# FutureSDR/FutureSDR

Hardware: NVIDIA H100
Metric: Msamples/s (higher is better)
Workload: dtype f32

## Files before the change

### futuresdr_b200/_lib.py

```python
from __future__ import annotations

import ctypes as C
import os

_HERE = os.path.dirname(os.path.abspath(__file__))
SO_PATH = os.environ.get("B2S_LIB") or os.path.join(_HERE, "libb200sdr.so")

OK, EINVAL, ECUDA, ENOMEM, EAGAIN, EUNSUPPORTED, ESTATE, ETIMEOUT = 0, -1, -2, -3, -4, -5, -6, -7
INSUFFICIENT_INPUT, INSUFFICIENT_OUTPUT, BOTH_SUFFICIENT = 0, 1, 2
F32_F32, C32_F32, C32_C32, F64_F64 = 0, 1, 2, 3
ALGO_AUTO, ALGO_DIRECT, ALGO_TENSOR, ALGO_FFT, ALGO_SCAN = 0, 1, 2, 3, 4
(OP_SCALE_F32, OP_SCALE_C32, OP_QUAD_DEMOD, OP_NORM_SQR, OP_QUAD_DEMOD_C32, OP_EXP_F32,
 OP_MAG_C32, OP_LOG10_F32, OP_DC_BLOCK_F32, OP_SLICE_F32_U8) = range(10)
KEYFOB_NONE, KEYFOB_CLOSE, KEYFOB_OPEN, KEYFOB_TRUNK = 0, 1, 2, 3
WAVE_COS, WAVE_SIN, WAVE_SQUARE = 0, 1, 2
(COMBINE_ADD_F32, COMBINE_SUB_F32, COMBINE_MUL_F32, COMBINE_CONJ_MUL_C32, COMBINE_MAG_DIV_C32_F32, COMBINE_TO_C32,
 COMBINE_TO_C32_NEG_Q) = range(7)
SPLIT_RE_IM, SPLIT_DUP_F32 = 0, 1
FANOUT_MAX_OUTPUTS = 256

_vp, _sz, _i32, _f32 = C.c_void_p, C.c_size_t, C.c_int32, C.c_float
_szp, _i32p, _vpp, _f32p = C.POINTER(C.c_size_t), C.POINTER(C.c_int32), C.POINTER(C.c_void_p), C.POINTER(C.c_float)

SIGNATURES = {
    "b2s_version": (_i32, []),
    "b2s_ctx_create": (_i32, [C.c_int, _vpp]),
    "b2s_ctx_create_on_stream": (_i32, [C.c_int, _vp, _vpp]),
    "b2s_ctx_destroy": (None, [_vp]),
    "b2s_last_error": (C.c_char_p, [_vp]),
    "b2s_ctx_sync": (_i32, [_vp]),
    "b2s_ctx_stream": (_vp, [_vp]),
    "b2s_ctx_sm_count": (_i32, [_vp]),
    "b2s_ctx_launch_count": (C.c_uint64, [_vp]),
    "b2s_ctx_bytes_held": (C.c_uint64, [_vp]),
    "b2s_malloc": (_i32, [_vp, _sz, _vpp]),
    "b2s_free": (_i32, [_vp, _vp]),
    "b2s_host_alloc": (_i32, [_vp, _sz, _vpp]),
    "b2s_host_free": (_i32, [_vp, _vp]),
    "b2s_memcpy_h2d": (_i32, [_vp, _vp, _vp, _sz]),
    "b2s_memcpy_d2h": (_i32, [_vp, _vp, _vp, _sz]),
    "b2s_fir_plan": (_i32, [_vp, C.c_int, _f32p, _sz, _sz, _vpp]),
    "b2s_fir_plan_f32_f32": (_i32, [_vp, _f32p, _sz, _sz, _vpp]),
    "b2s_fir_plan_c32_f32": (_i32, [_vp, _f32p, _sz, _sz, _vpp]),
    "b2s_fir_plan_c32_c32": (_i32, [_vp, _f32p, _sz, _sz, _vpp]),
    "b2s_fir_plan_f64_f64": (_i32, [_vp, C.POINTER(C.c_double), _sz, _sz, _vpp]),
    "b2s_fir_destroy": (None, [_vp]),
    "b2s_fir_length": (_sz, [_vp]),
    "b2s_fir_set_algo": (_i32, [_vp, C.c_int]),
    "b2s_fir_get_algo": (_i32, [_vp]),
    "b2s_fir_exec": (_i32, [_vp, _vp, _sz, _vp, _sz, _szp, _szp, _i32p]),
    "b2s_fir_filter_host": (_i32, [_vp, _vp, _sz, _vp, _sz, _szp, _szp, _i32p]),
    "b2s_fir_exec_hist": (_i32, [_vp, _vp, _sz, _vp, _sz, _vp, _sz, _vp, _szp, _szp, _i32p]),
    "b2s_resamp_plan": (_i32, [_vp, C.c_int, _f32p, _sz, _sz, _sz, _vpp]),
    "b2s_resamp_destroy": (None, [_vp]),
    "b2s_resamp_length": (_sz, [_vp]),
    "b2s_resamp_exec": (_i32, [_vp, _vp, _sz, _vp, _sz, _szp, _szp, _i32p]),
    "b2s_pfbarb_plan_c32": (_i32, [_vp, _f32p, _sz, _sz, _f32, _vpp]),
    "b2s_pfbarb_destroy": (None, [_vp]),
    "b2s_pfbarb_reset": (_i32, [_vp]),
    "b2s_pfbarb_period": (_i32, [_f32, _sz, C.POINTER(C.c_uint64), C.POINTER(C.c_uint64)]),
    "b2s_pfbarb_exec": (_i32, [_vp, _vp, _sz, _vp, _sz, _szp, _szp, _i32p]),
    "b2s_fft_plan_c32": (_i32, [_vp, _sz, _i32, _i32, _i32, _f32, _vpp]),
    "b2s_fft_destroy": (None, [_vp]),
    "b2s_fft_length": (_sz, [_vp]),
    "b2s_fft_exec": (_i32, [_vp, _vp, _sz, _vp, _sz, _szp, _szp]),
    "b2s_apply_create": (_i32, [_vp, C.c_int, _f32, _vpp]),
    "b2s_apply_destroy": (None, [_vp]),
    "b2s_apply_reset": (_i32, [_vp]),
    "b2s_apply_exec": (_i32, [_vp, _vp, _sz, _vp, _sz, _szp, _szp]),
    "b2s_rotator_create": (_i32, [_vp, _f32, _vpp]),
    "b2s_rotator_destroy": (None, [_vp]),
    "b2s_rotator_reset": (_i32, [_vp]),
    "b2s_rotator_exec": (_i32, [_vp, _vp, _sz, _vp, _sz, _szp, _i32p]),
    "b2s_xlating_taps": (_i32, [_f32p, _sz, _f32, _f32, _sz, _f32p, _f32p]),
    "b2s_chan_plan_c32": (_i32, [_vp, _sz, _f32p, _sz, _f32, _vpp]),
    "b2s_chan_destroy": (None, [_vp]),
    "b2s_chan_decimation": (_sz, [_vp]),
    "b2s_chan_exec": (_i32, [_vp, _vp, _sz, _vp, _sz, _sz, _szp, _szp, _i32p]),
    "b2s_synth_plan_c32": (_i32, [_vp, _sz, _f32p, _sz, _vpp]),
    "b2s_synth_destroy": (None, [_vp]),
    "b2s_synth_exec": (_i32, [_vp, _vp, _sz, _sz, _vp, _sz, _szp, _szp]),
    "b2s_mavg_create": (_i32, [_vp, _sz, _f32, _sz, _vpp]),
# ... 137 lines not shown
```

### futuresdr_b200/csrc/abi.cu

```cuda
#include <cmath>
#include <cstdlib>
#include <memory>

#include "fir.cuh"

thread_local std::string g_b2s_last_error;

int32_t b2s_fail(b2s_ctx *ctx, int32_t code, const char *fmt, ...) {
    char buf[512];
    va_list ap;
    va_start(ap, fmt);
    vsnprintf(buf, sizeof(buf), fmt, ap);
    va_end(ap);
    g_b2s_last_error = buf;
    if (ctx) ctx->err = buf;
    return code;
}

extern "C" {

int32_t b2s_version(void) { return B2S_VERSION; }

static int32_t ctx_create(int device, void *stream, bool own, b2s_ctx **out) {
    if (!out) return b2s_fail(nullptr, B2S_EINVAL, "b2s_ctx_create: out is NULL");
// ... 181 lines not shown
}
int32_t b2s_fir_plan_c32_f32(b2s_ctx *c, const float *t, size_t n, size_t d, b2s_fir **o) {
    return b2s_fir_plan(c, B2S_C32_F32, t, n, d, o);
}
int32_t b2s_fir_plan_c32_c32(b2s_ctx *c, const float *t, size_t n, size_t d, b2s_fir **o) {
    return b2s_fir_plan(c, B2S_C32_C32, t, n, d, o);
}

void b2s_fir_destroy(b2s_fir *f) { PlanDeleter<b2s_fir>()(f); }

size_t b2s_fir_length(const b2s_fir *f) { return f ? f->ntaps : 0; }

int32_t b2s_fir_set_algo(b2s_fir *f, b2s_algo algo) {
    if (!f) return b2s_fail(nullptr, B2S_EINVAL, "fir is NULL");
    if (algo < B2S_ALGO_AUTO || algo > B2S_ALGO_FFT)
        return b2s_fail(f->ctx, B2S_EUNSUPPORTED, "FIR filters have the AUTO, DIRECT, TENSOR and FFT algorithms (got %d)", (int)algo);
    if (f->kind == B2S_F64_F64)
        return algo == B2S_ALGO_AUTO || algo == B2S_ALGO_DIRECT ? B2S_OK
               : b2s_fail(f->ctx, B2S_EUNSUPPORTED, "f64 filters only have the CUDA-core form");
    if (algo == B2S_ALGO_TENSOR && !fir_tc_supported(f))
        return b2s_fail(f->ctx, B2S_EUNSUPPORTED,
                        "tensor algorithm needs real taps, 16..257 of them, and a decimation that divides 128 (kind %d, ntaps %zu, decim %zu)",
                        (int)f->kind, f->ntaps, f->decim);
    if (algo == B2S_ALGO_FFT && !fir_fft_supported(f))
        return b2s_fail(f->ctx, B2S_EUNSUPPORTED,
                        "FFT algorithm needs Complex<f32> samples, 64..2049 taps and decim == 1 (kind %d, ntaps %zu, decim %zu)",
                        (int)f->kind, f->ntaps, f->decim);
    f->algo_req = algo;
    resolve_algo(f);
    DeviceGuard g(f->ctx->device);
    return prepare_algo(f);
}
int32_t b2s_fir_get_algo(const b2s_fir *f) { return f ? (int32_t)f->algo : B2S_EINVAL; }

static void fir_counts(const b2s_fir *f, size_t n_in, size_t n_out_cap, size_t *consumed,
                       size_t *produced, int32_t *status) {
    const size_t filterable = sat_sub(n_in + 1, f->ntaps);
    const size_t consumable = filterable / f->decim;
    size_t n;
    int32_t st;
    if (consumable > n_out_cap) { n = n_out_cap; st = B2S_INSUFFICIENT_OUTPUT; }
    else if (consumable == n_out_cap) { n = n_out_cap; st = B2S_BOTH_SUFFICIENT; }
    else { n = consumable; st = B2S_INSUFFICIENT_INPUT; }
    *consumed = n * f->decim; *produced = n; *status = st;
}

static int32_t fir_launch(b2s_fir *f, const void *d_in, size_t n_in, void *d_out, size_t n_out,
                          cudaStream_t stream) {
    if (f->kind == B2S_F64_F64) return fir_f64_launch(f, d_in, n_in, d_out, n_out, stream);
    if (f->algo == B2S_ALGO_TENSOR && f->algo_req == B2S_ALGO_AUTO) {
        const double per_tap = f->kind == B2S_F32_F32 ? 6.9e-14 : 1.15e-13;
        if ((double)n_out * (double)f->ntaps * per_tap < 10e-6) return fir_direct_launch(f, d_in, n_in, d_out, n_out, stream);
    }
    if (f->algo == B2S_ALGO_TENSOR) return fir_tc_launch(f, d_in, n_in, d_out, n_out, stream);
    if (f->algo == B2S_ALGO_FFT) return fir_fft_launch(f, d_in, n_in, d_out, n_out, stream);
    return fir_direct_launch(f, d_in, n_in, d_out, n_out, stream);
}

int32_t b2s_fir_exec(b2s_fir *f, const void *d_in, size_t n_in, void *d_out, size_t n_out_cap,
                     size_t *consumed, size_t *produced, int32_t *status) {
    if (!f || !consumed || !produced || !status)
        return b2s_fail(f ? f->ctx : nullptr, B2S_EINVAL, "b2s_fir_exec: NULL argument");
    fir_counts(f, n_in, n_out_cap, consumed, produced, status);
    if (*produced == 0) return B2S_OK;
    if (!d_in || !d_out) return b2s_fail(f->ctx, B2S_EINVAL, "b2s_fir_exec: NULL buffer");
    DeviceGuard g(f->ctx->device);
// ... 118 lines not shown
```

### futuresdr_b200/csrc/fir.cuh

```cuda
#pragma once
#include "common.cuh"

struct b2s_fir {
    b2s_ctx *ctx = nullptr;
    b2s_kind kind = B2S_C32_F32;
    size_t ntaps = 0, decim = 1;
    std::vector<float> taps_host;
    b2s_algo algo_req = B2S_ALGO_AUTO, algo = B2S_ALGO_DIRECT;

    Buf<float> d_ptaps;
    int Upad = 0;

    int tc_kblocks = 0;
    bool tc_ready = false;
    int tc_flags = 0;

    Buf<float2> d_fftH;

    Buf<double> d_taps64;
};

int32_t fir_direct_prepare(b2s_fir *f);
int32_t fir_direct_launch(b2s_fir *f, const void *d_in, size_t n_in, void *d_out, size_t n_out,
                          cudaStream_t stream);
std::vector<float> slide_table(const float *taps, size_t tf, size_t L, size_t M, size_t T, size_t lead);
bool    resamp_slide_supported(size_t L, size_t M, size_t T, size_t item_bytes);
int32_t resamp_slide_launch(b2s_ctx *ctx, b2s_kind kind, const float *d_gtab, size_t L, size_t M, size_t T,
                            const void *d_in, size_t n_in, void *d_out, size_t n_out, cudaStream_t stream);
struct FirHist {
    const void *d_hist = nullptr;
    size_t n_hist = 0;
    unsigned *publish_flag = nullptr;
    unsigned publish_value = 0;
    const unsigned *wait_flag = nullptr;
    unsigned wait_value = 0;
    unsigned *done_flag = nullptr;
    unsigned done_value = 0;
};
bool    fir_tc_supported(const b2s_fir *f);
int32_t fir_tc_launch_hist(b2s_fir *f, const FirHist *h, const void *d_in, size_t n_in, void *d_out, size_t n_out,
                           cudaStream_t stream);
int32_t fir_tc_prepare(b2s_fir *f);
int32_t fir_tc_launch(b2s_fir *f, const void *d_in, size_t n_in, void *d_out, size_t n_out,
                      cudaStream_t stream);
int32_t fir_f64_prepare(b2s_fir *f, const double *taps);
int32_t fir_f64_launch(b2s_fir *f, const void *d_in, size_t n_in, void *d_out, size_t n_out, cudaStream_t stream);
bool    fir_fft_supported(const b2s_fir *f);
int32_t fir_fft_prepare(b2s_fir *f);
int32_t fir_fft_launch(b2s_fir *f, const void *d_in, size_t n_in, void *d_out, size_t n_out,
                       cudaStream_t stream);
```

### futuresdr_b200/csrc/fir_tc.cu

```cuda
#include <cuda_bf16.h>

#include <algorithm>
#include <climits>
#include <cstdlib>
#include <type_traits>

#include "fir.cuh"

namespace {

constexpr int kStages = 2;
#ifndef B2S_RAW_SLOTS
#define B2S_RAW_SLOTS 6
#endif
constexpr int kRawSlots = B2S_RAW_SLOTS;
constexpr int kRawSlotBytes = 8192;
constexpr int kNumProducerThreads = 256;
constexpr int kNumMathThreads = 256;
constexpr int kNumLoaderThreads = 128;
constexpr int kThreadsTC = kNumMathThreads + kNumProducerThreads + kNumLoaderThreads;
constexpr int kProdWarps = kNumProducerThreads / 32;
constexpr int kMathWarps = kNumMathThreads / 32;
constexpr int kProdWarp0 = kMathWarps;
constexpr int kTmaWarp = kProdWarp0 + kProdWarps;
constexpr int kRegsAtLaunch = 65536 / kThreadsTC / 8 * 8;
constexpr int kMathRegs = 176, kProdRegs = 48, kLoaderRegs = 24;
static_assert(kNumMathThreads * kMathRegs + kNumProducerThreads * kProdRegs + kNumLoaderThreads * kLoaderRegs <=
              kThreadsTC * kRegsAtLaunch, "setmaxnreg budget exceeds the CTA's register allocation");
constexpr int kAtomsOut = 16;
constexpr int kMaxDK = 3;
constexpr int kMaxKSteps = (63 + 128 * kMaxDK - 128) / 16 + 1;
constexpr int kSplitBytesMax = (kAtomsOut + kMaxDK - 1) * 1024 * 2;
constexpr int kStageBytes = 2 * kSplitBytesMax;
constexpr int kACores = kMaxDK * 16 + 15;
constexpr int kABytes = kACores * 128;
constexpr int kSmemTC = kStages * kStageBytes + kRawSlots * kRawSlotBytes + 2 * kABytes + 1024  + 256 ;
static_assert(kSmemTC <= 227 * 1024, "tensor FIR shared memory exceeds the 227 KiB per-CTA limit");

__device__ __forceinline__ uint32_t smem_u32(const void *p) { return (uint32_t)__cvta_generic_to_shared(p); }

__device__ __forceinline__ void mbar_init(uint32_t bar, uint32_t count) {
    asm volatile("mbarrier.init.shared::cta.b64 [%0], %1;" ::"r"(bar), "r"(count));
}
__device__ __forceinline__ void mbar_arrive(uint32_t bar) {
    asm volatile("mbarrier.arrive.shared::cta.b64 _, [%0];" ::"r"(bar) : "memory");
}
__device__ __forceinline__ bool mbar_try_wait(uint32_t bar, uint32_t parity) {
    uint32_t ok;
    asm volatile(
        "{\n\t.reg .pred p;\n\t"
        "mbarrier.try_wait.parity.shared::cta.b64 p, [%1], %2;\n\t"
        "selp.b32 %0, 1, 0, p;\n\t}"
        : "=r"(ok) : "r"(bar), "r"(parity) : "memory");
    return ok != 0;
}
__device__ __forceinline__ void mbar_wait(uint32_t bar, uint32_t parity) {
    while (!mbar_try_wait(bar, parity)) {}
}
__device__ __forceinline__ bool elect_one() {
    uint32_t pred;
    asm volatile("{\n\t.reg .pred p;\n\telect.sync _|p, 0xffffffff;\n\tselp.b32 %0, 1, 0, p;\n\t}" : "=r"(pred));
    return pred != 0;
}
__device__ __forceinline__ void fence_barrier_init() { asm volatile("fence.mbarrier_init.release.cluster;" ::: "memory"); }
__device__ __forceinline__ void fence_proxy_async() { asm volatile("fence.proxy.async.shared::cta;" ::: "memory"); }

__device__ __forceinline__ void wgmma_fence() { asm volatile("wgmma.fence.sync.aligned;" ::: "memory"); }
__device__ __forceinline__ void wgmma_commit() { asm volatile("wgmma.commit_group.sync.aligned;" ::: "memory"); }
__device__ __forceinline__ void wgmma_wait_all() { asm volatile("wgmma.wait_group.sync.aligned 0;" ::: "memory"); }
// ... 42 lines not shown
          "+f"(d[16]), "+f"(d[17]), "+f"(d[18]), "+f"(d[19]), "+f"(d[20]), "+f"(d[21]), "+f"(d[22]), "+f"(d[23]),
          "+f"(d[24]), "+f"(d[25]), "+f"(d[26]), "+f"(d[27]), "+f"(d[28]), "+f"(d[29]), "+f"(d[30]), "+f"(d[31]),
          "+f"(d[32]), "+f"(d[33]), "+f"(d[34]), "+f"(d[35]), "+f"(d[36]), "+f"(d[37]), "+f"(d[38]), "+f"(d[39]),
          "+f"(d[40]), "+f"(d[41]), "+f"(d[42]), "+f"(d[43]), "+f"(d[44]), "+f"(d[45]), "+f"(d[46]), "+f"(d[47]),
          "+f"(d[48]), "+f"(d[49]), "+f"(d[50]), "+f"(d[51]), "+f"(d[52]), "+f"(d[53]), "+f"(d[54]), "+f"(d[55]),
          "+f"(d[56]), "+f"(d[57]), "+f"(d[58]), "+f"(d[59]), "+f"(d[60]), "+f"(d[61]), "+f"(d[62]), "+f"(d[63])
        : "r"(a[0]), "r"(a[1]), "r"(a[2]), "r"(a[3]), "l"(b_desc), "r"(accumulate)
        : "memory");
}
__device__ __forceinline__ uint32_t ld_shared_b32(uint32_t addr) {
    uint32_t v;
    asm volatile("ld.shared.b32 %0, [%1];" : "=r"(v) : "r"(addr));
    return v;
}

__device__ __forceinline__ uint32_t cvt_bf16x2(float a, float b) {
    uint32_t r;
    asm("cvt.rn.bf16x2.f32 %0, %1, %2;" : "=r"(r) : "f"(b), "f"(a));
    return r;
}
__device__ __forceinline__ void split2(float a, float b, uint32_t &hi, uint32_t &lo) {
    hi = cvt_bf16x2(a, b);
    const float ah = __uint_as_float(hi << 16), bh = __uint_as_float(hi & 0xffff0000u);
    lo = cvt_bf16x2(a - ah, b - bh);
}

__device__ __forceinline__ uint64_t make_desc(uint32_t smem_addr, uint32_t lbo, uint32_t sbo, uint32_t layout) {
    return (uint64_t)((smem_addr & 0x3FFFF) >> 4) | ((uint64_t)(lbo >> 4) << 16) | ((uint64_t)(sbo >> 4) << 32) |
           ((uint64_t)layout << 62);
}
__device__ __forceinline__ uint64_t make_b_desc(uint32_t smem_addr) { return make_desc(smem_addr, 16, 1024, 1); }
__device__ __forceinline__ uint64_t make_a_desc(uint32_t smem_addr) { return make_desc(smem_addr, 128, 128, 0); }

struct TcParams {
    const float *in;
    float *out;
    const float *g;
    long long n_in;
    long long n_out;
    int ntaps;
    int DK;
    int num_tiles;
    int flags;
    int decim;
    const float *hist;
    int hist_items;
    int lead;
    const unsigned *wait_flag;
    unsigned wait_value;
    unsigned *done_flag;
    unsigned done_value;
    unsigned *pub_flag;
    unsigned pub_value;
    unsigned *status;
};

template <bool COMPLEX>
__global__ void __launch_bounds__(kThreadsTC, 1) fir_tc_kernel(const TcParams prm) {
    extern __shared__ unsigned char smem_raw[];
    const uint32_t raw = smem_u32(smem_raw);
    const uint32_t base = (raw + 1023u) & ~1023u;
    unsigned char *gen_base = smem_raw + (base - raw);
    const uint32_t raw_base = base + kStages * kStageBytes;
    unsigned char *raw_gen = gen_base + kStages * kStageBytes;
    const uint32_t a_base = raw_base + kRawSlots * kRawSlotBytes;
    __nv_bfloat16 *a_gen = reinterpret_cast<__nv_bfloat16 *>(raw_gen + kRawSlots * kRawSlotBytes);
    const uint32_t bar_base = a_base + 2 * kABytes;
    auto full_bar = [&](int s) { return bar_base + 8u * s; };
    auto empty_bar = [&](int s) { return bar_base + 8u * (kStages + s); };
    auto rfull_bar = [&](int r) { return bar_base + 8u * (2 * kStages + r); };
    auto rempty_bar = [&](int r) { return bar_base + 8u * (2 * kStages + kRawSlots + r); };

    const int warp = threadIdx.x >> 5, lane = threadIdx.x & 31;
    if (prm.pub_flag && blockIdx.x == 0 && threadIdx.x == 0) {
        __threadfence_system();
        asm volatile("st.release.sys.global.u32 [%0], %1;" ::"l"(prm.pub_flag), "r"(prm.pub_value) : "memory");
    }
    const int DK = prm.DK, K = 128 * DK;
    const int atoms = kAtomsOut + DK - 1;
    const int chunk_bytes = atoms * 1024;
    const int split_bytes = 2 * chunk_bytes;
    constexpr int NSEQ = COMPLEX ? 4 : 8;
    constexpr int TILE_BLOCKS = kAtomsOut * NSEQ;
    constexpr long long TILE_ITEMS = (long long)TILE_BLOCKS * 128;

    if (warp == kTmaWarp && lane == 0) {
        for (int s = 0; s < kStages; s++) { mbar_init(full_bar(s), kProdWarps); mbar_init(empty_bar(s), kMathWarps); }
        for (int r = 0; r < kRawSlots; r++) { mbar_init(rfull_bar(r), 1); mbar_init(rempty_bar(r), kProdWarps); }
        fence_barrier_init();
    }
    const int a_elems = (K / 8 + 15) * 64;
    for (int i = threadIdx.x; i < a_elems; i += kThreadsTC) {
        const int s = i >> 6, r = (i >> 3) & 7, e = i & 7;
        const int t = 8 * s + r + e - 127 - prm.lead;
        const float gv = (t >= 0 && t < prm.ntaps) ? __ldg(prm.g + t) : 0.0f;
        const __nv_bfloat16 hi = __float2bfloat16_rn(gv);
        a_gen[i] = hi;
        a_gen[kABytes / 2 + i] = __float2bfloat16_rn(gv - __bfloat162float(hi));
    }
    fence_proxy_async();
    __syncthreads();

    constexpr int F4_PER_BLOCK = COMPLEX ? 64 : 32;
    constexpr int BLOCKS_PER_SLOT = 512 / F4_PER_BLOCK;
    constexpr int SLOTS_PER_TILE = (TILE_BLOCKS + kMaxDK - 1 + BLOCKS_PER_SLOT - 1) / BLOCKS_PER_SLOT;
    constexpr int ITEM_BYTES = COMPLEX ? 8 : 4;
    const int in_blocks = TILE_BLOCKS + DK - 1;

    if (warp >= kTmaWarp) {
        setmaxnreg_dec<kLoaderRegs>();
        if (warp != kTmaWarp) return;
        if (elect_one()) {
            int rs = 0;
            uint32_t rphase = 0;
            for (int tile = blockIdx.x; tile < prm.num_tiles; tile += gridDim.x) {
                const long long item0 = (long long)tile * TILE_ITEMS;
#pragma unroll 1
                for (int s = 0; s < SLOTS_PER_TILE; s++) {
                    const int blk_first = s * BLOCKS_PER_SLOT;
                    if (blk_first >= in_blocks) break;
                    const int nblk = min(BLOCKS_PER_SLOT, in_blocks - blk_first);
                    const long long it0 = item0 + (long long)blk_first * 128;
                    long long items = (long long)nblk * 128;
                    if (it0 + items > prm.n_in) items = prm.n_in - it0;
                    long long bytes = items > 0 ? ((items * ITEM_BYTES) & ~15ll) : 0;
                    mbar_wait(rempty_bar(rs), rphase ^ 1);
                    if (tile == 0 && s == 0 && prm.hist_items > 0) {
                        if (prm.wait_flag) {
                            unsigned long long t0, t1;
                            asm volatile("mov.u64 %0, %%globaltimer;" : "=l"(t0));
                            for (;;) {
                                unsigned v;
                                asm volatile("ld.acquire.sys.global.u32 %0, [%1];" : "=r"(v) : "l"(prm.wait_flag) : "memory");
                                if ((int)(v - prm.wait_value) >= 0) break;
                                asm volatile("mov.u64 %0, %%globaltimer;" : "=l"(t1));
                                if (t1 - t0 > 4000000000ull) { atomicOr(prm.status, 1u); break; }
                                __nanosleep(64);
                            }
                            asm volatile("fence.proxy.async;" ::: "memory");
                        }
                        const uint32_t hb = (uint32_t)prm.hist_items * ITEM_BYTES;
                        const uint32_t rest = bytes > (long long)hb ? (uint32_t)bytes - hb : 0u;
                        asm volatile("mbarrier.arrive.expect_tx.shared::cta.b64 _, [%0], %1;" ::"r"(rfull_bar(rs)), "r"(hb + rest) : "memory");
                        asm volatile("cp.async.bulk.shared::cluster.global.mbarrier::complete_tx::bytes [%0], [%1], %2, [%3];"
                                     ::"r"(raw_base + rs * kRawSlotBytes), "l"(prm.hist), "r"(hb), "r"(rfull_bar(rs)) : "memory");
                        if (rest)
                            asm volatile("cp.async.bulk.shared::cluster.global.mbarrier::complete_tx::bytes [%0], [%1], %2, [%3];"
                                         ::"r"(raw_base + rs * kRawSlotBytes + hb), "l"(prm.in + (COMPLEX ? 2 : 1) * (long long)prm.hist_items),
                                           "r"(rest), "r"(rfull_bar(rs)) : "memory");
                    } else if (bytes > 0) {
                        asm volatile("mbarrier.arrive.expect_tx.shared::cta.b64 _, [%0], %1;" ::"r"(rfull_bar(rs)), "r"((uint32_t)bytes) : "memory");
                        asm volatile("cp.async.bulk.shared::cluster.global.mbarrier::complete_tx::bytes [%0], [%1], %2, [%3];"
                                     ::"r"(raw_base + rs * kRawSlotBytes), "l"(prm.in + (COMPLEX ? 2 : 1) * it0),
                                       "r"((uint32_t)bytes), "r"(rfull_bar(rs)) : "memory");
                    } else {
                        mbar_arrive(rfull_bar(rs));
                    }
                    if (++rs == kRawSlots) { rs = 0; rphase ^= 1; }
                }
            }
        }
        __syncwarp();
    } else if (warp >= kProdWarp0) {
        setmaxnreg_dec<kProdRegs>();
        const int tid = threadIdx.x - 32 * kProdWarp0;
        const int fo = tid % F4_PER_BLOCK, rowsel = tid / F4_PER_BLOCK;
        const int kc = COMPLEX ? (fo >> 5) : (fo >> 4);
        const int c16 = COMPLEX ? ((fo & 31) >> 2) : ((fo & 15) >> 1);
        const int wofs = COMPLEX ? (fo & 3) * 4 : (fo & 1) * 8;
        const uint32_t t_off = (uint32_t)(kc * chunk_bytes + wofs + rowsel * 1024);
        uint32_t xj[8];
#pragma unroll
        for (int j = 0; j < 8; j++) xj[j] = (uint32_t)(j * 128 + ((c16 ^ j) << 4));
        const bool alias_thread = rowsel < DK - 1;
        const uint32_t sb = (uint32_t)split_bytes;

        auto convert_tile = [&](auto interior_c, unsigned char *stage_ptr, long long item0, int &rs, uint32_t &rphase) {
            constexpr bool INTERIOR = decltype(interior_c)::value;
            unsigned char *tp = stage_ptr + t_off;
#pragma unroll
            for (int s = 0; s < SLOTS_PER_TILE; s++) {
                if (s * BLOCKS_PER_SLOT >= in_blocks) break;
                mbar_wait(rfull_bar(rs), rphase);
                const float4 *raw = reinterpret_cast<const float4 *>(raw_gen + rs * kRawSlotBytes);
                float4 v[2];
                v[0] = raw[tid];
                v[1] = raw[tid + 256];
                const int rs_cur = rs;
                if (++rs == kRawSlots) { rs = 0; rphase ^= 1; }
                if constexpr (!INTERIOR) {
                    if (s == 0 && item0 == 0 && tid == 0 && prm.done_flag)
// ... 33 lines not shown
                            *reinterpret_cast<uint32_t *>(q + xj[2 * (seq & 3) + 1]) = ih;
                            *reinterpret_cast<uint32_t *>(q + xj[2 * (seq & 3) + 1] + sb) = il;
                        }
                        if (alias_ct && alias_thread) {
                            unsigned char *q = tp + (g_ct + kAtomsOut) * 1024;
                            *reinterpret_cast<uint32_t *>(q + xj[2 * ((seq - 1) & 3)]) = rh;
                            *reinterpret_cast<uint32_t *>(q + xj[2 * ((seq - 1) & 3)] + sb) = rl;
                            *reinterpret_cast<uint32_t *>(q + xj[2 * ((seq - 1) & 3) + 1]) = ih;
                            *reinterpret_cast<uint32_t *>(q + xj[2 * ((seq - 1) & 3) + 1] + sb) = il;
                        }
                    } else {
                        uint32_t h0, l0, h1, l1;
                        split2(v[i].x, v[i].y, h0, l0);
                        split2(v[i].z, v[i].w, h1, l1);
                        if (seq < NSEQ) {
                            unsigned char *q = tp + g_ct * 1024 + xj[seq & 7];
                            *reinterpret_cast<uint2 *>(q) = make_uint2(h0, h1);
                            *reinterpret_cast<uint2 *>(q + sb) = make_uint2(l0, l1);
                        }
                        if (alias_ct && alias_thread) {
                            unsigned char *q = tp + (g_ct + kAtomsOut) * 1024 + xj[(seq - 1) & 7];
                            *reinterpret_cast<uint2 *>(q) = make_uint2(h0, h1);
                            *reinterpret_cast<uint2 *>(q + sb) = make_uint2(l0, l1);
                        }
                    }
                }
                __syncwarp();
                if (lane == 0) mbar_arrive(rempty_bar(rs_cur));
            }
        };

        int stage = 0, rs = 0;
        uint32_t phase = 0, rphase = 0;
        for (int tile = blockIdx.x; tile < prm.num_tiles; tile += gridDim.x) {
            const long long item0 = (long long)tile * TILE_ITEMS;
            const bool interior = item0 + (long long)in_blocks * 128 <= prm.n_in &&
                                  !(tile == 0 && (prm.lead | prm.hist_items) != 0);
            mbar_wait(empty_bar(stage), phase ^ 1);
            unsigned char *stage_ptr = gen_base + stage * kStageBytes;
            if (interior) convert_tile(std::true_type{}, stage_ptr, item0, rs, rphase);
            else convert_tile(std::false_type{}, stage_ptr, item0, rs, rphase);
            fence_proxy_async();
            __syncwarp();
            if (lane == 0) mbar_arrive(full_bar(stage));
            if (++stage == kStages) { stage = 0; phase ^= 1; }
        }
    } else {
        setmaxnreg_inc<kMathRegs>();
        const int wg = __shfl_sync(0xffffffffu, warp >> 2, 0);
        const int wl = warp & 3, q4 = lane & 3;
        const int D = prm.decim, per_blk = 128 / D;
        const uint32_t a_hi = a_base + 1024u * wg, a_lo = a_hi + kABytes;
        const int p0 = 64 * (1 - wg);
        const int j0 = p0 / 16;
        const int nsteps = (prm.flags & 4) ? 0 : min((p0 + 63 + prm.lead + prm.ntaps - 1) / 16, 8 * DK - 1) - j0 + 1;

        uint32_t ghi[kMaxKSteps][4];
        {
            const uint32_t f0 = a_hi + 256u * (uint32_t)(wl + j0) + 16u * (uint32_t)(lane >> 2) + 4u * (uint32_t)q4;
#pragma unroll
            for (int i = 0; i < kMaxKSteps; i++) {
                const uint32_t f = f0 + 256u * i;
                const bool used = i < nsteps;
                ghi[i][0] = used ? ld_shared_b32(f) : 0u;
                ghi[i][1] = used ? ld_shared_b32(f + 128u) : 0u;
                ghi[i][2] = used ? ld_shared_b32(f + 128u) : 0u;
                ghi[i][3] = used ? ld_shared_b32(f + 256u) : 0u;
            }
        }

        const uint64_t a_lo_desc = make_a_desc(a_lo + 256u * j0);

        int stage = 0;
        uint32_t phase = 0;
        auto mma_tile = [&](float (&acc)[64]) {
            mbar_wait(full_bar(stage), phase);
            wgmma_fence();
            const uint64_t b_desc = make_b_desc(base + stage * kStageBytes);
#pragma unroll
            for (int i = 0; i < kMaxKSteps; i++) {
                if (i >= nsteps) break;
                const int m = (j0 >> 2) + (i >> 2);
                const uint64_t bh = b_desc + (uint32_t)(((m & 1) * chunk_bytes + (m >> 1) * 1024 + (i & 3) * 32) >> 4);
                wgmma_m64n128_rs(acc, ghi[i], bh, i != 0);
                wgmma_m64n128_rs(acc, ghi[i], bh + (uint32_t)(split_bytes >> 4), 1u);
                wgmma_m64n128(acc, a_lo_desc + 16u * i, bh, 1u);
            }
            wgmma_commit();
        };
        auto release_stage = [&]() {
            wgmma_wait_all();
            __syncwarp();
            if (lane == 0) mbar_arrive(empty_bar(stage));
            if (++stage == kStages) { stage = 0; phase ^= 1; }
        };
        const int log2D = __ffs(D) - 1;
        auto store_tile = [&](const float (&acc)[64], int tile) {
            if (prm.flags & 2) return;
#pragma unroll
            for (int h = 0; h < 2; h++) {
                const int p = 127 - (64 * wg + 16 * wl + (lane >> 2) + 8 * h);
                const int keep = (p & (D - 1)) == D - 1;
                const long long kb = ((long long)tile * TILE_BLOCKS + kAtomsOut * q4 * (COMPLEX ? 1 : 2)) * per_blk +
                                     (p >> log2D);
                const int room = (int)max(min(prm.n_out - kb, (long long)INT_MAX), 0ll) & -keep;
                const int ncols = (int)(((unsigned)room + (unsigned)per_blk - 1u) >> (7 - log2D));
                if constexpr (COMPLEX) {
#pragma unroll
                    for (int gam = 0; gam < 16; gam++)
                        st_global_if(reinterpret_cast<float2 *>(prm.out) + kb + gam * per_blk, acc[4 * gam + 2 * h],
                                     acc[4 * gam + 2 * h + 1], gam < ncols);
                } else {
#pragma unroll
                    for (int n = 0; n < 2 * kAtomsOut; n++)
                        st_global_if(prm.out + (kb + n * per_blk), acc[4 * (n % kAtomsOut) + 2 * h + n / kAtomsOut],
                                     n < ncols);
                }
            }
        };

        float acc[64];
#pragma unroll
        for (int i = 0; i < 64; i++) acc[i] = 0.0f;
        for (int tile = blockIdx.x; tile < prm.num_tiles; tile += gridDim.x) {
            mma_tile(acc);
            release_stage();
            store_tile(acc, tile);
        }
    }
}

}

bool fir_tc_supported(const b2s_fir *f) {
    if (f->decim == 0 || f->decim > 128 || 128 % f->decim != 0) return false;
    if (f->kind != B2S_C32_F32 && f->kind != B2S_F32_F32) return false;
    return f->ntaps >= 16 && f->ntaps <= 128 * kMaxDK - 127;
}

int32_t fir_tc_prepare(b2s_fir *f) {
    b2s_ctx *ctx = f->ctx;
    if (f->tc_ready) return B2S_OK;
    if (!fir_tc_supported(f)) return b2s_fail(ctx, B2S_EUNSUPPORTED, "tensor FIR: unsupported plan");
    f->tc_kblocks = (int)ceil_div(f->ntaps + 127, 128);
    B2S_CUDA(ctx, cudaFuncSetAttribute(fir_tc_kernel<true>, cudaFuncAttributeMaxDynamicSharedMemorySize, kSmemTC));
    B2S_CUDA(ctx, cudaFuncSetAttribute(fir_tc_kernel<false>, cudaFuncAttributeMaxDynamicSharedMemorySize, kSmemTC));
    for (const void *k : {(const void *)fir_tc_kernel<true>, (const void *)fir_tc_kernel<false>}) {
        cudaFuncAttributes attr;
        B2S_CUDA(ctx, cudaFuncGetAttributes(&attr, k));
        if (attr.numRegs != kRegsAtLaunch)
            return b2s_fail(ctx, B2S_EUNSUPPORTED, "tensor FIR: kernel built with %d registers per thread, its setmaxnreg "
                            "budget assumes %d", attr.numRegs, kRegsAtLaunch);
    }
    if (const char *e = getenv("B2S_TC_FLAGS")) f->tc_flags = atoi(e);
    f->tc_ready = true;
    return B2S_OK;
}

int32_t fir_tc_launch_hist(b2s_fir *f, const FirHist *h, const void *d_in, size_t n_in, void *d_out, size_t n_out,
                           cudaStream_t stream) {
    b2s_ctx *ctx = f->ctx;
    if (n_out == 0) return B2S_OK;
    if (!f->tc_ready) return b2s_fail(ctx, B2S_ESTATE, "tensor FIR not prepared");
    const bool cplx = f->kind == B2S_C32_F32;
    const size_t item = cplx ? 8 : 4, q = 16 / item;
    const uintptr_t a_in = reinterpret_cast<uintptr_t>(d_in), a_out = reinterpret_cast<uintptr_t>(d_out);
    if ((a_in % item) || (a_out % item)) return B2S_EAGAIN;
    const size_t n_hist = h ? h->n_hist : 0;
    size_t lead;
    if (n_hist) {
        const uintptr_t a_h = reinterpret_cast<uintptr_t>(h->d_hist);
        if ((a_h % item) || (a_in & 15)) return B2S_EAGAIN;
        lead = (a_h / item) % q;
        if ((lead + n_hist) % q) return B2S_EAGAIN;
        if (lead + n_hist > 1024 || n_in * item < 16) return B2S_EAGAIN;
    } else {
        lead = (a_in / item) % q;
    }
    const int DK = (int)ceil_div(f->ntaps + lead + 127, 128);
    if (DK > kMaxDK) return B2S_EAGAIN;
    TcParams prm;
    prm.lead = (int)lead;
    prm.hist_items = n_hist ? (int)(lead + n_hist) : 0;
    prm.hist = n_hist ? (const float *)h->d_hist - lead * (item / 4) : nullptr;
    prm.in = (const float *)d_in - (lead + n_hist) * (item / 4);
    prm.wait_flag = (h && n_hist) ? h->wait_flag : nullptr;
    prm.wait_value = h ? h->wait_value : 0;
    prm.done_flag = (h && n_hist) ? h->done_flag : nullptr;
    prm.done_value = h ? h->done_value : 0;
    prm.pub_flag = h ? h->publish_flag : nullptr;
    prm.pub_value = h ? h->publish_value : 0;
    prm.status = ctx->d_status;
    prm.out = (float *)d_out;
    prm.g = f->d_ptaps.get() + (size_t)f->decim * f->Upad;
    prm.n_in = (long long)(lead + n_hist + n_in);
    prm.n_out = (long long)n_out;
    prm.decim = (int)f->decim;
    prm.ntaps = (int)f->ntaps;
    prm.DK = DK;
    const long long tile_items = cplx ? 64 * 128 : 128 * 128;
    prm.num_tiles = (int)ceil_div(n_out * f->decim, (size_t)tile_items);
    prm.flags = f->tc_flags;
    const int grid = std::min(prm.num_tiles, ctx->sm_count);
    if (prm.wait_flag) ctx->flag_ops++;
    if (cplx) fir_tc_kernel<true><<<grid, kThreadsTC, kSmemTC, stream>>>(prm);
    else fir_tc_kernel<false><<<grid, kThreadsTC, kSmemTC, stream>>>(prm);
    B2S_CHECK_LAUNCH(ctx);
    return B2S_OK;
}

int32_t fir_tc_launch(b2s_fir *f, const void *d_in, size_t n_in, void *d_out, size_t n_out,
                      cudaStream_t stream) {
    const int32_t rc = fir_tc_launch_hist(f, nullptr, d_in, n_in, d_out, n_out, stream);
    if (rc == B2S_EAGAIN) return fir_direct_launch(f, d_in, n_in, d_out, n_out, stream);
    return rc;
}
```

### include/b200sdr.h

```cpp
#ifndef B200SDR_H
#define B200SDR_H

#include <stddef.h>
#include <stdint.h>

#ifdef __cplusplus
extern "C" {
#endif

#define B2S_VERSION 100

#define B2S_OK            0
#define B2S_EINVAL       (-1)
#define B2S_ECUDA        (-2)
#define B2S_ENOMEM       (-3)
#define B2S_EAGAIN       (-4)
#define B2S_EUNSUPPORTED (-5)
#define B2S_ESTATE       (-6)
#define B2S_ETIMEOUT     (-7)

#define B2S_INSUFFICIENT_INPUT  0
#define B2S_INSUFFICIENT_OUTPUT 1
#define B2S_BOTH_SUFFICIENT     2

// ... 19 lines not shown
typedef struct b2s_fft    b2s_fft;
typedef struct b2s_apply  b2s_apply;
typedef struct b2s_ring   b2s_ring;
typedef struct b2s_slot   b2s_slot;

int32_t     b2s_version(void);
int32_t     b2s_ctx_create(int device, b2s_ctx **out);
int32_t     b2s_ctx_create_on_stream(int device, void *stream, b2s_ctx **out);
void        b2s_ctx_destroy(b2s_ctx *ctx);
const char *b2s_last_error(const b2s_ctx *ctx);
int32_t     b2s_ctx_sync(b2s_ctx *ctx);
void       *b2s_ctx_stream(b2s_ctx *ctx);
int32_t     b2s_ctx_sm_count(b2s_ctx *ctx);
uint64_t    b2s_ctx_launch_count(const b2s_ctx *ctx);
uint64_t    b2s_ctx_bytes_held(const b2s_ctx *ctx);

int32_t b2s_malloc(b2s_ctx *ctx, size_t bytes, void **dptr);
int32_t b2s_free(b2s_ctx *ctx, void *dptr);
int32_t b2s_host_alloc(b2s_ctx *ctx, size_t bytes, void **hptr);
int32_t b2s_host_free(b2s_ctx *ctx, void *hptr);
int32_t b2s_memcpy_h2d(b2s_ctx *ctx, void *dptr, const void *hptr, size_t bytes);
int32_t b2s_memcpy_d2h(b2s_ctx *ctx, void *hptr, const void *dptr, size_t bytes);

int32_t b2s_fir_plan(b2s_ctx *ctx, b2s_kind kind, const float *taps, size_t ntaps, size_t decim,
                     b2s_fir **out);
int32_t b2s_fir_plan_f32_f32(b2s_ctx *ctx, const float *taps, size_t ntaps, size_t decim, b2s_fir **out);
int32_t b2s_fir_plan_c32_f32(b2s_ctx *ctx, const float *taps, size_t ntaps, size_t decim, b2s_fir **out);
int32_t b2s_fir_plan_c32_c32(b2s_ctx *ctx, const float *taps, size_t ntaps, size_t decim, b2s_fir **out);
int32_t b2s_fir_plan_f64_f64(b2s_ctx *ctx, const double *taps, size_t ntaps, size_t decim, b2s_fir **out);
void    b2s_fir_destroy(b2s_fir *f);
size_t  b2s_fir_length(const b2s_fir *f);
int32_t b2s_fir_set_algo(b2s_fir *f, b2s_algo algo);
int32_t b2s_fir_get_algo(const b2s_fir *f);

int32_t b2s_fir_exec(b2s_fir *f, const void *d_in, size_t n_in, void *d_out, size_t n_out_cap,
                     size_t *consumed, size_t *produced, int32_t *status);
typedef struct b2s_handshake {
    uint32_t       *publish_flag; uint32_t publish_value;
    const uint32_t *wait_flag;    uint32_t wait_value;
    uint32_t       *done_flag;    uint32_t done_value;
} b2s_handshake;
int32_t b2s_fir_exec_hist(b2s_fir *f, const void *d_hist, size_t n_hist, const void *d_in, size_t n_in,
                          void *d_out, size_t n_out_cap, const b2s_handshake *hs, size_t *consumed, size_t *produced,
                          int32_t *status);
int32_t b2s_fir_filter_host(b2s_fir *f, const void *h_in, size_t n_in, void *h_out, size_t n_out_cap,
                            size_t *consumed, size_t *produced, int32_t *status);

int32_t b2s_resamp_plan(b2s_ctx *ctx, b2s_kind kind, const float *taps, size_t ntaps, size_t interp,
                        size_t decim, b2s_resamp **out);
void    b2s_resamp_destroy(b2s_resamp *r);
size_t  b2s_resamp_length(const b2s_resamp *r);
int32_t b2s_resamp_exec(b2s_resamp *r, const void *d_in, size_t n_in, void *d_out, size_t n_out_cap,
                        size_t *consumed, size_t *produced, int32_t *status);

int32_t b2s_pfbarb_plan_c32(b2s_ctx *ctx, const float *taps, size_t ntaps, size_t num_filters,
                            float rate, b2s_pfbarb **out);
void    b2s_pfbarb_destroy(b2s_pfbarb *p);
int32_t b2s_pfbarb_reset(b2s_pfbarb *p);
int32_t b2s_pfbarb_period(float rate, size_t num_filters, uint64_t *period_items, uint64_t *outputs_per_period);
int32_t b2s_pfbarb_exec(b2s_pfbarb *p, const void *d_in, size_t n_in, void *d_out, size_t n_out_cap,
                        size_t *consumed, size_t *produced, int32_t *call_again);

int32_t b2s_fft_plan_c32(b2s_ctx *ctx, size_t n, int32_t inverse, int32_t fft_shift,
                         int32_t has_normalize, float normalize, b2s_fft **out);
void    b2s_fft_destroy(b2s_fft *f);
size_t  b2s_fft_length(const b2s_fft *f);
// ... 213 lines not shown
```

Before: 169,700.

## Schedule tensor FIR tiles dynamically via global atomic counter and prefetch first slots

```diff
diff --git a/futuresdr_b200/_lib.py b/futuresdr_b200/_lib.py
--- a/futuresdr_b200/_lib.py
+++ b/futuresdr_b200/_lib.py
@@ -48,6 +48,7 @@
     "b2s_fir_length": (_sz, [_vp]),
     "b2s_fir_set_algo": (_i32, [_vp, C.c_int]),
     "b2s_fir_get_algo": (_i32, [_vp]),
+    "b2s_fir_tc_timeline": (_i32, [_vp, C.POINTER(C.c_uint64), _sz, _szp]),
     "b2s_fir_exec": (_i32, [_vp, _vp, _sz, _vp, _sz, _szp, _szp, _i32p]),
     "b2s_fir_filter_host": (_i32, [_vp, _vp, _sz, _vp, _sz, _szp, _szp, _i32p]),
     "b2s_fir_exec_hist": (_i32, [_vp, _vp, _sz, _vp, _sz, _vp, _sz, _vp, _szp, _szp, _i32p]),
diff --git a/futuresdr_b200/csrc/abi.cu b/futuresdr_b200/csrc/abi.cu
--- a/futuresdr_b200/csrc/abi.cu
+++ b/futuresdr_b200/csrc/abi.cu
@@ -237,6 +237,11 @@
     return prepare_algo(f);
 }
 int32_t b2s_fir_get_algo(const b2s_fir *f) { return f ? (int32_t)f->algo : B2S_EINVAL; }
+
+int32_t b2s_fir_tc_timeline(b2s_fir *f, uint64_t *stamps, size_t cap, size_t *n_ctas) {
+    if (!f || !stamps || !n_ctas) return b2s_fail(f ? f->ctx : nullptr, B2S_EINVAL, "b2s_fir_tc_timeline: NULL argument");
+    return fir_tc_timeline(f, stamps, cap, n_ctas);
+}
 
 static void fir_counts(const b2s_fir *f, size_t n_in, size_t n_out_cap, size_t *consumed,
                        size_t *produced, int32_t *status) {
diff --git a/futuresdr_b200/csrc/fir.cuh b/futuresdr_b200/csrc/fir.cuh
--- a/futuresdr_b200/csrc/fir.cuh
+++ b/futuresdr_b200/csrc/fir.cuh
@@ -14,6 +14,9 @@
     int tc_kblocks = 0;
     bool tc_ready = false;
     int tc_flags = 0;
+    Buf<unsigned> d_tc_sched;
+    Buf<unsigned long long> d_tc_timeline;
+    int tc_timeline_ctas = 0;
 
     Buf<float2> d_fftH;
 
@@ -37,10 +40,12 @@
     unsigned *done_flag = nullptr;
     unsigned done_value = 0;
 };
+enum TcStamp { kTcEntry, kTcFirstCopy, kTcFirstFull, kTcLastTile, kTcExit, kTcTiles, kTcStampWords };
 bool    fir_tc_supported(const b2s_fir *f);
 int32_t fir_tc_launch_hist(b2s_fir *f, const FirHist *h, const void *d_in, size_t n_in, void *d_out, size_t n_out,
                            cudaStream_t stream);
 int32_t fir_tc_prepare(b2s_fir *f);
+int32_t fir_tc_timeline(b2s_fir *f, uint64_t *stamps, size_t cap, size_t *n_ctas);
 int32_t fir_tc_launch(b2s_fir *f, const void *d_in, size_t n_in, void *d_out, size_t n_out,
                       cudaStream_t stream);
 int32_t fir_f64_prepare(b2s_fir *f, const double *taps);
diff --git a/futuresdr_b200/csrc/fir_tc.cu b/futuresdr_b200/csrc/fir_tc.cu
--- a/futuresdr_b200/csrc/fir_tc.cu
+++ b/futuresdr_b200/csrc/fir_tc.cu
@@ -34,7 +34,9 @@
 constexpr int kStageBytes = 2 * kSplitBytesMax;
 constexpr int kACores = kMaxDK * 16 + 15;
 constexpr int kABytes = kACores * 128;
+constexpr int kTileRing = 8;
 constexpr int kSmemTC = kStages * kStageBytes + kRawSlots * kRawSlotBytes + 2 * kABytes + 1024  + 256 ;
+static_assert(8 * (2 * kStages + 2 * kRawSlots) + 4 * kTileRing <= 256, "barriers and tile ring exceed their 256 bytes");
 static_assert(kSmemTC <= 227 * 1024, "tensor FIR shared memory exceeds the 227 KiB per-CTA limit");
 
 __device__ __forceinline__ uint32_t smem_u32(const void *p) { return (uint32_t)__cvta_generic_to_shared(p); }
@@ -143,6 +145,12 @@
 __device__ __forceinline__ uint64_t make_b_desc(uint32_t smem_addr) { return make_desc(smem_addr, 16, 1024, 1); }
 __device__ __forceinline__ uint64_t make_a_desc(uint32_t smem_addr) { return make_desc(smem_addr, 128, 128, 0); }
 
+__device__ __forceinline__ unsigned long long globaltimer() {
+    unsigned long long t;
+    asm volatile("mov.u64 %0, %%globaltimer;" : "=l"(t));
+    return t;
+}
+
 struct TcParams {
     const float *in;
     float *out;
@@ -153,6 +161,8 @@
     int DK;
     int num_tiles;
     int flags;
+    unsigned long long *timeline;
+    unsigned *sched;
     int decim;
     const float *hist;
     int hist_items;
@@ -181,8 +191,12 @@
     auto empty_bar = [&](int s) { return bar_base + 8u * (kStages + s); };
     auto rfull_bar = [&](int r) { return bar_base + 8u * (2 * kStages + r); };
     auto rempty_bar = [&](int r) { return bar_base + 8u * (2 * kStages + kRawSlots + r); };
+    const uint32_t tile_ring = bar_base + 8u * (2 * kStages + 2 * kRawSlots);
+    auto tile_at = [&](int j) { return (int)ld_shared_b32(tile_ring + 4u * (uint32_t)(j & (kTileRing - 1))); };
 
     const int warp = threadIdx.x >> 5, lane = threadIdx.x & 31;
+    unsigned long long *const stamps = prm.timeline ? prm.timeline + (size_t)blockIdx.x * kTcStampWords : nullptr;
+    if (stamps && threadIdx.x == 0) stamps[kTcEntry] = globaltimer();
     if (prm.pub_flag && blockIdx.x == 0 && threadIdx.x == 0) {
         __threadfence_system();
         asm volatile("st.release.sys.global.u32 [%0], %1;" ::"l"(prm.pub_flag), "r"(prm.pub_value) : "memory");
@@ -195,10 +209,66 @@
     constexpr int TILE_BLOCKS = kAtomsOut * NSEQ;
     constexpr long long TILE_ITEMS = (long long)TILE_BLOCKS * 128;
 
-    if (warp == kTmaWarp && lane == 0) {
-        for (int s = 0; s < kStages; s++) { mbar_init(full_bar(s), kProdWarps); mbar_init(empty_bar(s), kMathWarps); }
-        for (int r = 0; r < kRawSlots; r++) { mbar_init(rfull_bar(r), 1); mbar_init(rempty_bar(r), kProdWarps); }
-        fence_barrier_init();
+    constexpr int F4_PER_BLOCK = COMPLEX ? 64 : 32;
+    constexpr int BLOCKS_PER_SLOT = 512 / F4_PER_BLOCK;
+    constexpr int SLOTS_PER_TILE = (TILE_BLOCKS + kMaxDK - 1 + BLOCKS_PER_SLOT - 1) / BLOCKS_PER_SLOT;
+    constexpr int ITEM_BYTES = COMPLEX ? 8 : 4;
+    const int in_blocks = TILE_BLOCKS + DK - 1;
+    const int tile_slots = (in_blocks + BLOCKS_PER_SLOT - 1) / BLOCKS_PER_SLOT;
+    const int pre_slots = min(kRawSlots, tile_slots);
+
+    auto load_slot = [&](int tile, int s, int rs, uint32_t rphase) {
+        const long long item0 = (long long)tile * TILE_ITEMS;
+        const int blk_first = s * BLOCKS_PER_SLOT;
+        const int nblk = min(BLOCKS_PER_SLOT, in_blocks - blk_first);
+        const long long it0 = item0 + (long long)blk_first * 128;
+        long long items = (long long)nblk * 128;
+        if (it0 + items > prm.n_in) items = prm.n_in - it0;
+        long long bytes = items > 0 ? ((items * ITEM_BYTES) & ~15ll) : 0;
+        mbar_wait(rempty_bar(rs), rphase ^ 1);
+        if (tile == 0 && s == 0 && prm.hist_items > 0) {
+            if (prm.wait_flag) {
+                unsigned long long t0, t1;
+                asm volatile("mov.u64 %0, %%globaltimer;" : "=l"(t0));
+                for (;;) {
+                    unsigned v;
+                    asm volatile("ld.acquire.sys.global.u32 %0, [%1];" : "=r"(v) : "l"(prm.wait_flag) : "memory");
+                    if ((int)(v - prm.wait_value) >= 0) break;
+                    asm volatile("mov.u64 %0, %%globaltimer;" : "=l"(t1));
+                    if (t1 - t0 > 4000000000ull) { atomicOr(prm.status, 1u); break; }
+                    __nanosleep(64);
+                }
+                asm volatile("fence.proxy.async;" ::: "memory");
+            }
+            const uint32_t hb = (uint32_t)prm.hist_items * ITEM_BYTES;
+            const uint32_t rest = bytes > (long long)hb ? (uint32_t)bytes - hb : 0u;
+            asm volatile("mbarrier.arrive.expect_tx.shared::cta.b64 _, [%0], %1;" ::"r"(rfull_bar(rs)), "r"(hb + rest) : "memory");
+            asm volatile("cp.async.bulk.shared::cluster.global.mbarrier::complete_tx::bytes [%0], [%1], %2, [%3];"
+                         ::"r"(raw_base + rs * kRawSlotBytes), "l"(prm.hist), "r"(hb), "r"(rfull_bar(rs)) : "memory");
+            if (rest)
+                asm volatile("cp.async.bulk.shared::cluster.global.mbarrier::complete_tx::bytes [%0], [%1], %2, [%3];"
+                             ::"r"(raw_base + rs * kRawSlotBytes + hb), "l"(prm.in + (COMPLEX ? 2 : 1) * (long long)prm.hist_items),
+                               "r"(rest), "r"(rfull_bar(rs)) : "memory");
+        } else if (bytes > 0) {
+            asm volatile("mbarrier.arrive.expect_tx.shared::cta.b64 _, [%0], %1;" ::"r"(rfull_bar(rs)), "r"((uint32_t)bytes) : "memory");
+            asm volatile("cp.async.bulk.shared::cluster.global.mbarrier::complete_tx::bytes [%0], [%1], %2, [%3];"
+                         ::"r"(raw_base + rs * kRawSlotBytes), "l"(prm.in + (COMPLEX ? 2 : 1) * it0),
+                           "r"((uint32_t)bytes), "r"(rfull_bar(rs)) : "memory");
+        } else {
+            mbar_arrive(rfull_bar(rs));
+        }
+        if (stamps && tile == blockIdx.x && s == 0) stamps[kTcFirstCopy] = globaltimer();
+    };
+
+    if (warp == kTmaWarp) {
+        if (elect_one()) {
+            for (int s = 0; s < kStages; s++) { mbar_init(full_bar(s), kProdWarps); mbar_init(empty_bar(s), kMathWarps); }
+            for (int r = 0; r < kRawSlots; r++) { mbar_init(rfull_bar(r), 1); mbar_init(rempty_bar(r), kProdWarps); }
+            fence_barrier_init();
+            asm volatile("st.shared.b32 [%0], %1;" ::"r"(tile_ring), "r"((int)blockIdx.x) : "memory");
+            for (int s = 0; s < pre_slots; s++) load_slot(blockIdx.x, s, s, 0u);
+        }
+        __syncwarp();
     }
     const int a_elems = (K / 8 + 15) * 64;
     for (int i = threadIdx.x; i < a_elems; i += kThreadsTC) {
@@ -212,62 +282,32 @@
     fence_proxy_async();
     __syncthreads();
 
-    constexpr int F4_PER_BLOCK = COMPLEX ? 64 : 32;
-    constexpr int BLOCKS_PER_SLOT = 512 / F4_PER_BLOCK;
-    constexpr int SLOTS_PER_TILE = (TILE_BLOCKS + kMaxDK - 1 + BLOCKS_PER_SLOT - 1) / BLOCKS_PER_SLOT;
-    constexpr int ITEM_BYTES = COMPLEX ? 8 : 4;
-    const int in_blocks = TILE_BLOCKS + DK - 1;
-
     if (warp >= kTmaWarp) {
         setmaxnreg_dec<kLoaderRegs>();
         if (warp != kTmaWarp) return;
         if (elect_one()) {
-            int rs = 0;
-            uint32_t rphase = 0;
-            for (int tile = blockIdx.x; tile < prm.num_tiles; tile += gridDim.x) {
-                const long long item0 = (long long)tile * TILE_ITEMS;
+            int rs = pre_slots % kRawSlots;
+            uint32_t rphase = pre_slots / kRawSlots;
+            for (int j = 0, tile = blockIdx.x, s0 = pre_slots;; s0 = 0) {
+                const int next = (int)gridDim.x + (int)atomicAdd(prm.sched, 1u);
 #pragma unroll 1
-                for (int s = 0; s < SLOTS_PER_TILE; s++) {
-                    const int blk_first = s * BLOCKS_PER_SLOT;
-                    if (blk_first >= in_blocks) break;
-                    const int nblk = min(BLOCKS_PER_SLOT, in_blocks - blk_first);
-                    const long long it0 = item0 + (long long)blk_first * 128;
-                    long long items = (long long)nblk * 128;
-                    if (it0 + items > prm.n_in) items = prm.n_in - it0;
-                    long long bytes = items > 0 ? ((items * ITEM_BYTES) & ~15ll) : 0;
+                for (int s = s0; s < tile_slots; s++) {
+                    load_slot(tile, s, rs, rphase);
+                    if (++rs == kRawSlots) { rs = 0; rphase ^= 1; }
+                }
+                tile = next;
+                j++;
+                asm volatile("st.shared.b32 [%0], %1;" ::"r"(tile_ring + 4u * (uint32_t)(j & (kTileRing - 1))),
+                             "r"(tile < prm.num_tiles ? tile : -1) : "memory");
+                if (tile >= prm.num_tiles) {
                     mbar_wait(rempty_bar(rs), rphase ^ 1);
-                    if (tile == 0 && s == 0 && prm.hist_items > 0) {
-                        if (prm.wait_flag) {
-                            unsigned long long t0, t1;
-                            asm volatile("mov.u64 %0, %%globaltimer;" : "=l"(t0));
-                            for (;;) {
-                                unsigned v;
-                                asm volatile("ld.acquire.sys.global.u32 %0, [%1];" : "=r"(v) : "l"(prm.wait_flag) : "memory");
-                                if ((int)(v - prm.wait_value) >= 0) break;
-                                asm volatile("mov.u64 %0, %%globaltimer;" : "=l"(t1));
-                                if (t1 - t0 > 4000000000ull) { atomicOr(prm.status, 1u); break; }
-                                __nanosleep(64);
-                            }
-                            asm volatile("fence.proxy.async;" ::: "memory");
-                        }
-                        const uint32_t hb = (uint32_t)prm.hist_items * ITEM_BYTES;
-                        const uint32_t rest = bytes > (long long)hb ? (uint32_t)bytes - hb : 0u;
-                        asm volatile("mbarrier.arrive.expect_tx.shared::cta.b64 _, [%0], %1;" ::"r"(rfull_bar(rs)), "r"(hb + rest) : "memory");
-                        asm volatile("cp.async.bulk.shared::cluster.global.mbarrier::complete_tx::bytes [%0], [%1], %2, [%3];"
-                                     ::"r"(raw_base + rs * kRawSlotBytes), "l"(prm.hist), "r"(hb), "r"(rfull_bar(rs)) : "memory");
-                        if (rest)
-                            asm volatile("cp.async.bulk.shared::cluster.global.mbarrier::complete_tx::bytes [%0], [%1], %2, [%3];"
-                                         ::"r"(raw_base + rs * kRawSlotBytes + hb), "l"(prm.in + (COMPLEX ? 2 : 1) * (long long)prm.hist_items),
-                                           "r"(rest), "r"(rfull_bar(rs)) : "memory");
-                    } else if (bytes > 0) {
-                        asm volatile("mbarrier.arrive.expect_tx.shared::cta.b64 _, [%0], %1;" ::"r"(rfull_bar(rs)), "r"((uint32_t)bytes) : "memory");
-                        asm volatile("cp.async.bulk.shared::cluster.global.mbarrier::complete_tx::bytes [%0], [%1], %2, [%3];"
-                                     ::"r"(raw_base + rs * kRawSlotBytes), "l"(prm.in + (COMPLEX ? 2 : 1) * it0),
-                                       "r"((uint32_t)bytes), "r"(rfull_bar(rs)) : "memory");
-                    } else {
-                        mbar_arrive(rfull_bar(rs));
+                    mbar_arrive(rfull_bar(rs));
+                    __threadfence();
+                    if (atomicAdd(prm.sched + 1, 1u) == gridDim.x - 1) {
+                        prm.sched[0] = 0;
+                        prm.sched[1] = 0;
                     }
-                    if (++rs == kRawSlots) { rs = 0; rphase ^= 1; }
+                    break;
                 }
             }
         }
@@ -367,11 +407,18 @@
 
         int stage = 0, rs = 0;
         uint32_t phase = 0, rphase = 0;
-        for (int tile = blockIdx.x; tile < prm.num_tiles; tile += gridDim.x) {
+        for (int j = 0;; j++) {
+            mbar_wait(rfull_bar(rs), rphase);
+            const int tile = tile_at(j);
+            mbar_wait(empty_bar(stage), phase ^ 1);
+            if (tile < 0) {
+                __syncwarp();
+                if (lane == 0) mbar_arrive(full_bar(stage));
+                break;
+            }
             const long long item0 = (long long)tile * TILE_ITEMS;
             const bool interior = item0 + (long long)in_blocks * 128 <= prm.n_in &&
                                   !(tile == 0 && (prm.lead | prm.hist_items) != 0);
-            mbar_wait(empty_bar(stage), phase ^ 1);
             unsigned char *stage_ptr = gen_base + stage * kStageBytes;
             if (interior) convert_tile(std::true_type{}, stage_ptr, item0, rs, rphase);
             else convert_tile(std::false_type{}, stage_ptr, item0, rs, rphase);
@@ -409,7 +456,6 @@
         int stage = 0;
         uint32_t phase = 0;
         auto mma_tile = [&](float (&acc)[64]) {
-            mbar_wait(full_bar(stage), phase);
             wgmma_fence();
             const uint64_t b_desc = make_b_desc(base + stage * kStageBytes);
 #pragma unroll
@@ -457,10 +503,24 @@
         float acc[64];
 #pragma unroll
         for (int i = 0; i < 64; i++) acc[i] = 0.0f;
-        for (int tile = blockIdx.x; tile < prm.num_tiles; tile += gridDim.x) {
+        int tiles = 0;
+        unsigned long long t_last = 0;
+        for (;; tiles++) {
+            mbar_wait(full_bar(stage), phase);
+            const int tile = __shfl_sync(0xffffffffu, tile_at(tiles), 0);
+            if (tile < 0) break;
+            if (stamps && threadIdx.x == 0) {
+                t_last = globaltimer();
+                if (tiles == 0) stamps[kTcFirstFull] = t_last;
+            }
             mma_tile(acc);
             release_stage();
             store_tile(acc, tile);
+        }
+        if (stamps && threadIdx.x == 0) {
+            stamps[kTcLastTile] = t_last;
+            stamps[kTcExit] = globaltimer();
+            stamps[kTcTiles] = (unsigned long long)tiles;
         }
     }
 }
@@ -488,6 +548,9 @@
                             "budget assumes %d", attr.numRegs, kRegsAtLaunch);
     }
     if (const char *e = getenv("B2S_TC_FLAGS")) f->tc_flags = atoi(e);
+    B2S_TRY(f->d_tc_sched.alloc(ctx, 2, "tensor FIR tile counter"));
+    B2S_CUDA(ctx, cudaMemsetAsync(f->d_tc_sched.get(), 0, 2 * sizeof(unsigned), ctx->stream));
+    B2S_CUDA(ctx, cudaStreamSynchronize(ctx->stream));
     f->tc_ready = true;
     return B2S_OK;
 }
@@ -537,6 +600,15 @@
     prm.num_tiles = (int)ceil_div(n_out * f->decim, (size_t)tile_items);
     prm.flags = f->tc_flags;
     const int grid = std::min(prm.num_tiles, ctx->sm_count);
+    prm.sched = f->d_tc_sched.get();
+    prm.timeline = nullptr;
+    if (prm.flags & 16) {
+        const size_t words = (size_t)grid * kTcStampWords;
+        if (f->d_tc_timeline.size() < words) B2S_TRY(f->d_tc_timeline.alloc(ctx, words, "tensor FIR timeline"));
+        B2S_CUDA(ctx, cudaMemsetAsync(f->d_tc_timeline.get(), 0, words * sizeof(unsigned long long), stream));
+        prm.timeline = f->d_tc_timeline.get();
+        f->tc_timeline_ctas = grid;
+    }
     if (prm.wait_flag) ctx->flag_ops++;
     if (cplx) fir_tc_kernel<true><<<grid, kThreadsTC, kSmemTC, stream>>>(prm);
     else fir_tc_kernel<false><<<grid, kThreadsTC, kSmemTC, stream>>>(prm);
@@ -544,6 +616,18 @@
     return B2S_OK;
 }
 
+int32_t fir_tc_timeline(b2s_fir *f, uint64_t *stamps, size_t cap, size_t *n_ctas) {
+    b2s_ctx *ctx = f->ctx;
+    *n_ctas = 0;
+    if (!f->d_tc_timeline) return b2s_fail(ctx, B2S_ESTATE, "tensor FIR: no timeline recorded (B2S_TC_FLAGS bit 16)");
+    const size_t words = (size_t)f->tc_timeline_ctas * kTcStampWords;
+    if (cap < words) return b2s_fail(ctx, B2S_EINVAL, "tensor FIR timeline: %zu words needed, room for %zu", words, cap);
+    B2S_CUDA(ctx, cudaDeviceSynchronize());
+    B2S_CUDA(ctx, cudaMemcpy(stamps, f->d_tc_timeline.get(), words * sizeof(uint64_t), cudaMemcpyDeviceToHost));
+    *n_ctas = (size_t)f->tc_timeline_ctas;
+    return B2S_OK;
+}
+
 int32_t fir_tc_launch(b2s_fir *f, const void *d_in, size_t n_in, void *d_out, size_t n_out,
                       cudaStream_t stream) {
     const int32_t rc = fir_tc_launch_hist(f, nullptr, d_in, n_in, d_out, n_out, stream);
diff --git a/include/b200sdr.h b/include/b200sdr.h
--- a/include/b200sdr.h
+++ b/include/b200sdr.h
@@ -75,6 +75,7 @@
 size_t  b2s_fir_length(const b2s_fir *f);
 int32_t b2s_fir_set_algo(b2s_fir *f, b2s_algo algo);
 int32_t b2s_fir_get_algo(const b2s_fir *f);
+int32_t b2s_fir_tc_timeline(b2s_fir *f, uint64_t *stamps, size_t cap, size_t *n_ctas);
 
 int32_t b2s_fir_exec(b2s_fir *f, const void *d_in, size_t n_in, void *d_out, size_t n_out_cap,
                      size_t *consumed, size_t *produced, int32_t *status);
```

After: 170,200 (median of 6 runs). About the same (+0.3%).
